# mathwrx/Decouple-and-Couple_Learning_in_Multi-Modal_Brain_Tumor_Segmentation

Hardware: AMD Instinct MI355X
Metric: training volumes/sec (4x128^3) (higher is better)
Workload: dtype bf16x3 forward (split-bf16 MFMA operands hi.hi+hi.lo+lo.hi: logits within 1e-3 of the fp32 reference) / bf16 data-gradient / bf16 weight-gradient MFMA operands; f32 accumulate, f32 storage, f32 master weights

## Files before the change

### decouple-and-couple_learning_in_multi-modal_brain_tumor_segmentation_amd/csrc/conv_args.h

```cpp
#pragma once
#include "common.h"

typedef __bf16 bf16x8 __attribute__((ext_vector_type(8)));
typedef unsigned u32x4 __attribute__((ext_vector_type(4)));

struct ConvArgsB {
  ConvGeom g;
  const float* x; const uint4* wpk; const float* bias; float* y;
  const float* in_scale; const float* in_shift; float in_slope;
  const float* residual; int r_ldc; const float* out_scale; double* stats;
  unsigned long long unused_[2];
  const float* nb_x; int nb_ldc; const float* nb_scale; const float* nb_shift; float nb_slope;
  int groups, x_goff, y_goff;
  const uint4* wpk_g[3]; const float* bias_g[3];
  const uint4* x16; const uint4* zero16;
  unsigned short* y16;
};

typedef __bf16 bf16x2_t __attribute__((ext_vector_type(2)));
typedef float f32x2_t __attribute__((ext_vector_type(2)));
__device__ __forceinline__ unsigned pack_bf16(float a, float b) {
  const f32x2_t f = {a, b};
  return __builtin_bit_cast(unsigned, __builtin_convertvector(f, bf16x2_t));
}
__device__ __forceinline__ float bf16_round(float a) { return (float)(__bf16)a; }
__device__ __forceinline__ void split_bf16(float a, float b, unsigned& hi, unsigned& lo) {
  hi = pack_bf16(a, b);
  const float ha = __builtin_bit_cast(float, hi << 16), hb = __builtin_bit_cast(float, hi & 0xffff0000u);
  lo = pack_bf16(a - ha, b - hb);
}
__device__ __forceinline__ float act01(float v, float slope) { return fmaxf(v, v * slope); }


static inline int cfg_extent(int op, int Di, int Hi, int Wi, int Do, int Ho, int Wo, int cd[3]) {
  cd[0] = Do; cd[1] = Ho; cd[2] = Wo;
  if (op == CWF_CONVT2) { cd[0] = Di; cd[1] = Hi; cd[2] = Wi; return 8; }
  if (op == CWF_CONV3_S2_DGRAD) { cd[0] = (Do + 1) / 2; cd[1] = (Ho + 1) / 2; cd[2] = (Wo + 1) / 2; return 8; }
  return 1;
}

int cwf_try_conv_ws(int op, int x3, ConvArgsB& a, hipStream_t st, int* rc);
int cwf_ws_takes_x3();
int cwf_try_conv_wsp(int op, int x3, int cfg_mt, int cfg_wm, ConvArgsB& a, hipStream_t st, int* rc);

int conv_fp32_launch(const cwf_conv_args& d, hipStream_t st);
int conv_stem_launch(const cwf_conv_args& d, hipStream_t st);
int conv_s2c16_launch(const cwf_conv_args& d, hipStream_t st);
int wgrad_fp32_launch(const cwf_wgrad_args& d, int* nsplit_used, hipStream_t st);
```

### decouple-and-couple_learning_in_multi-modal_brain_tumor_segmentation_amd/csrc/conv_ws.hip

```cpp
#include "conv_args.h"
#include <cstdlib>
#include <type_traits>

#define WS_ID 6
#define WS_IH 6
#define WS_IW 18
#define WS_NVOX (WS_ID * WS_IH * WS_IW)
#define WS_SLOTS 11
#define WS_NT 2

struct WsWork { int ngroups, slots, tiles, xcd_perm; };

__host__ __device__ constexpr int ws_tap_bytes(int t) { return (((t / 9) * WS_IH + (t / 3) % 3) * WS_IW + t % 3) * 32; }

template <bool X3>
__global__ __launch_bounds__(512) void convws_kernel(const ConvArgsB a, const WsWork wk) {
  constexpr int NT = WS_NT;
  constexpr int T = 1;
  extern __shared__ float4 lds4[];
  const ConvGeom& g = a.g;
  const int nch = g.nchunks;
  char* lds = reinterpret_cast<char*>(lds4);
  constexpr int B_IMG = 14 * NT * 1024;
  constexpr int B_ALL = B_IMG * (X3 ? 2 : 1);
  constexpr int A_IMG = WS_NVOX * 32;
  constexpr int A_GRP = A_IMG * (X3 ? 2 : 1);
  constexpr int NB = (B_ALL + 4095) / 4096;
  char* Bh = lds;
  char* Bl = lds + B_IMG;
  const int tid = threadIdx.x, lane = tid & 63;
  const int wave = __builtin_amdgcn_readfirstlane(tid >> 6);
  const int grp = wave >> 2, wl = wave & 3, tg = tid & 255;
  char* Ah = lds + B_ALL + grp * A_GRP;
  char* Al = Ah + A_IMG;
  float* red = reinterpret_cast<float*>(lds + B_ALL + 2 * A_GRP);
  const int r = lane & 15, kq = lane >> 4;
  const bool second = (kq >> 1) != 0;

  int cgrp, slot;
  {
    const int b = blockIdx.x;
    if (wk.xcd_perm) {
      const int per = gridDim.x >> 3, j = b >> 3;
      cgrp = j % wk.ngroups;
      slot = (b & 7) * (per / wk.ngroups) + j / wk.ngroups;
    } else {
      cgrp = b % wk.ngroups;
      slot = b / wk.ngroups;
    }
  }
  const int t_begin = (int)(((int64_t)slot * wk.tiles) / wk.slots), t_end = (int)(((int64_t)(slot + 1) * wk.tiles) / wk.slots);
  const int nt0 = cgrp * NT;
  const int n_rounds = (t_end - t_begin + 2 * T - 1) / (2 * T);
  const int n_blocks = n_rounds * nch;
  const int tiles_per_n = g.tiles_d * g.tiles_h * g.tiles_w;
  auto item_tile = [&](int round, int k) { const int t = t_begin + round * 2 * T + 2 * k + grp; return t < t_end ? t : -1; };

  u32x4 bpf[NB];
  const uint4* wsrc = a.wpk + (int64_t)g.cls_wbase16[0] * 128;
  auto b_issue = [&](int chunk) {
    int tgo = tg;
    asm volatile("" : "+v"(tgo));
#pragma unroll
    for (int i = 0; i < NB; ++i) {
      int e = tgo + 256 * i;
      if (e >= B_ALL / 16) e = 0;
      const int img = e / (14 * NT * 64), e2 = e % (14 * NT * 64);
      const int ln = e2 & 63, blk = e2 >> 6;
      const int j = blk % NT, s = blk / NT;
      const uint4* p = wsrc + ((int64_t)(chunk * 14 + s) * g.ntiles + nt0 + j) * 128 + ln * 2 + img;
      bpf[i] = *reinterpret_cast<const u32x4*>(p);
    }
  };
  auto b_write = [&]() {
    int wb = tg * 16;
    asm volatile("" : "+v"(wb));
#pragma unroll
    for (int i = 0; i < NB; ++i)
      if (256 * (i + 1) <= B_ALL / 16 || tg + 256 * i < B_ALL / 16) *reinterpret_cast<u32x4*>(Bh + wb + i * 4096) = bpf[i];
  };

  const int q = tg & 3;
  const int vox0 = tg >> 2;
  const int iw_0 = vox0 % WS_IW, row_0 = vox0 / WS_IW;
  const bool plain = a.in_scale == nullptr && a.in_slope == 1.f;

  f32x4 pf[WS_SLOTS];
  f32x4 pf_sc, pf_sh;
  unsigned pf_inb = 0u;
  auto issue_loads = [&](int tile, int chunk) {
    const int n = tile / tiles_per_n;
    int bx = tile - n * tiles_per_n;
    const int tw = bx % g.tiles_w; bx /= g.tiles_w;
    const int th = bx % g.tiles_h, td = bx / g.tiles_h;
    const int id0 = td * 4 - 1, ih0 = th * 4 - 1, iw0 = tw * 16 - 1;
    const float* xb = a.x + (int64_t)n * g.Di * g.Hi * g.Wi * g.x_ldc + chunk * 16;
    const unsigned ldc4 = (unsigned)g.x_ldc * 4u;
    pf_inb = 0u;
    int iw = iw_0, row = row_0;
    asm volatile("" : "+v"(iw), "+v"(row));
#pragma unroll
    for (int i = 0; i < WS_SLOTS; ++i) {
      const int idd = (row * 43) >> 8, ih = row - idd * WS_IH;
      const int gd = id0 + idd, gh = ih0 + ih, gw = iw0 + iw;
      const bool ok = (row < WS_ID * WS_IH) & ((unsigned)gd < (unsigned)g.Di) & ((unsigned)gh < (unsigned)g.Hi) & ((unsigned)gw < (unsigned)g.Wi);
      iw += 10; row += 3;
      if (iw >= WS_IW) { iw -= WS_IW; ++row; }
      const unsigned lin = (unsigned)((gd * g.Hi + gh) * g.Wi + gw) * ldc4 + (unsigned)q * 16u;
      const unsigned boff = ok ? lin : (unsigned)q * 16u;
      pf[i] = *reinterpret_cast<const f32x4*>(reinterpret_cast<const char*>(xb) + boff);
      pf_inb |= ok ? (1u << i) : 0u;
    }
    const float* scp = a.in_scale ? a.in_scale + (int64_t)n * g.Cin + chunk * 16 : a.x;
    const float* shp = a.in_scale ? a.in_shift + (int64_t)n * g.Cin + chunk * 16 : a.x;
    const unsigned qo = (unsigned)q * 16u;
    pf_sc = *reinterpret_cast<const f32x4*>(reinterpret_cast<const char*>(scp) + qo);
    pf_sh = *reinterpret_cast<const f32x4*>(reinterpret_cast<const char*>(shp) + qo);
  };
  auto convert_write = [&](int tile, int chunk, const f32x4& sc, const f32x4& sh) {
    const float slope = a.in_slope;
    int vbase = (tg >> 2) * 32 + q * 8;
    asm volatile("" : "+v"(vbase));
#pragma unroll
    for (int i = 0; i < WS_SLOTS; ++i) {
      if (i == WS_SLOTS - 1 && vox0 + 64 * i >= WS_NVOX) continue;
      float v0 = pf[i][0], v1 = pf[i][1], v2 = pf[i][2], v3 = pf[i][3];
      if (!plain) {
        v0 = act01(fmaf(v0, sc[0], sh[0]), slope); v1 = act01(fmaf(v1, sc[1], sh[1]), slope);
        v2 = act01(fmaf(v2, sc[2], sh[2]), slope); v3 = act01(fmaf(v3, sc[3], sh[3]), slope);
      }
      uint2 h, l;
      if (X3) { split_bf16(v0, v1, h.x, l.x); split_bf16(v2, v3, h.y, l.y); }
      else { h.x = pack_bf16(v0, v1); h.y = pack_bf16(v2, v3); l = make_uint2(0u, 0u); }
      const bool was = (pf_inb >> i) & 1u;
      h.x = was ? h.x : 0u; h.y = was ? h.y : 0u; l.x = was ? l.x : 0u; l.y = was ? l.y : 0u;
      *reinterpret_cast<uint2*>(Ah + vbase + i * (64 * 32)) = h;
      if (X3) *reinterpret_cast<uint2*>(Al + vbase + i * (64 * 32)) = l;
    }
  };

  const int a_lane = ((wl * WS_IH) * WS_IW + r) * 32 + (kq & 1) * 16;
  const int b_lane = lane * 16;

  f32x4 acc[T][4][NT];
#pragma unroll
  for (int k = 0; k < T; ++k)
#pragma unroll
    for (int m = 0; m < 4; ++m)
#pragma unroll
      for (int j = 0; j < NT; ++j) acc[k][m][j] = (f32x4){0.f, 0.f, 0.f, 0.f};
  float s1[NT], s2[NT];
#pragma unroll
  for (int j = 0; j < NT; ++j) { s1[j] = 0.f; s2[j] = 0.f; }
  int stats_n = -1;

  auto flush_stats_wave = [&]() {
#pragma unroll
    for (int j = 0; j < NT; ++j) {
      float u1 = s1[j], u2 = s2[j];
      u1 += __shfl_xor(u1, 16, 64); u1 += __shfl_xor(u1, 32, 64);
      u2 += __shfl_xor(u2, 16, 64); u2 += __shfl_xor(u2, 32, 64);
      if (kq == 0) {
        const int co = (nt0 + j) * 16 + r;
        atomic_add_f64(a.stats + ((int64_t)stats_n * g.Cout + co) * 2 + 0, (double)u1);
        atomic_add_f64(a.stats + ((int64_t)stats_n * g.Cout + co) * 2 + 1, (double)u2);
      }
      s1[j] = 0.f; s2[j] = 0.f;
    }
  };

  auto epilogue = [&](int tile, auto KK) {
    constexpr int k = decltype(KK)::value;
    const int n = tile / tiles_per_n;
    int bx = tile - n * tiles_per_n;
    const int tw = bx % g.tiles_w; bx /= g.tiles_w;
    const int th = bx % g.tiles_h, td = bx / g.tiles_h;
    if (a.stats && n != stats_n) {
      if (stats_n >= 0) flush_stats_wave();
      stats_n = n;
    }
    float bvj[NT];
#pragma unroll
    for (int j = 0; j < NT; ++j) bvj[j] = a.bias ? a.bias[(nt0 + j) * 16 + r] : 0.f;
    auto epi = [&](auto HR, auto HT, auto HN) {
      constexpr bool HAS_RES = decltype(HR)::value, HAS_STATS = decltype(HT)::value, HAS_NB = decltype(HN)::value;
      unsigned yo[4], ro[4], xo[4];
      float nsc[NT], nsh[NT];
#pragma unroll
      for (int i = 0; i < 4; ++i) {
        yo[i] = (unsigned)((kq * 4 + i) * g.y_ldc + nt0 * 16 + r) * 4u; asm volatile("" : "+v"(yo[i]));
        if (HAS_RES) { ro[i] = (unsigned)((kq * 4 + i) * a.r_ldc + nt0 * 16 + r) * 4u; asm volatile("" : "+v"(ro[i])); }
        if (HAS_NB) { xo[i] = (unsigned)((kq * 4 + i) * a.nb_ldc + nt0 * 16 + r) * 4u; asm volatile("" : "+v"(xo[i])); }
      }
      if (HAS_NB) {
#pragma unroll
        for (int j = 0; j < NT; ++j) {
          nsc[j] = a.nb_scale[(int64_t)n * g.Cout + (nt0 + j) * 16 + r];
          nsh[j] = a.nb_shift[(int64_t)n * g.Cout + (nt0 + j) * 16 + r];
        }
      }
#pragma unroll
      for (int m = 0; m < 4; ++m) {
        const int od = td * 4 + wl, oh = th * 4 + m;
        const int64_t vox0 = (((int64_t)n * g.Do + od) * g.Ho + oh) * g.Wo + tw * 16;
        char* yb = reinterpret_cast<char*>(a.y + vox0 * g.y_ldc);
        const char* rb = HAS_RES ? reinterpret_cast<const char*>(a.residual + vox0 * a.r_ldc) : nullptr;
        const char* xb = HAS_NB ? reinterpret_cast<const char*>(a.nb_x + vox0 * a.nb_ldc) : nullptr;
        float rv[NT][4], xv[NT][4];
        if (HAS_RES) {
#pragma unroll
          for (int j = 0; j < NT; ++j)
#pragma unroll
            for (int i = 0; i < 4; ++i) rv[j][i] = *reinterpret_cast<const float*>(rb + ro[i] + j * 64);
        }
        if (HAS_NB) {
#pragma unroll
          for (int j = 0; j < NT; ++j)
#pragma unroll
            for (int i = 0; i < 4; ++i) xv[j][i] = *reinterpret_cast<const float*>(xb + xo[i] + j * 64);
        }
#pragma unroll
        for (int j = 0; j < NT; ++j)
#pragma unroll
          for (int i = 0; i < 4; ++i) {
            float v = acc[k][m][j][i] + bvj[j];
            if (HAS_RES) v += rv[j][i];
            *reinterpret_cast<float*>(yb + yo[i] + j * 64) = v;
            if (HAS_NB) {
              const float h = fmaf(xv[j][i], nsc[j], nsh[j]);
              const float gn = v * (h > 0.f ? 1.f : a.nb_slope);
              s1[j] += gn; s2[j] = fmaf(gn, h, s2[j]);
            } else if (HAS_STATS) { s1[j] += v; s2[j] = fmaf(v, v, s2[j]); }
            acc[k][m][j][i] = 0.f;
          }
      }
    };
    using T_ = std::true_type; using F_ = std::false_type;
    if (a.nb_x) { if (a.residual) epi(T_{}, T_{}, T_{}); else epi(F_{}, T_{}, T_{}); }
    else if (a.residual) { if (a.stats) epi(T_{}, T_{}, F_{}); else epi(T_{}, F_{}, F_{}); }
    else            { if (a.stats) epi(F_{}, T_{}, F_{}); else epi(F_{}, F_{}, F_{}); }
  };

  auto mfma_item = [&](int block, auto KK) -> bool {
    constexpr int k = decltype(KK)::value;
    const int round = block / nch, chunk = block - round * nch;
    const int tile = item_tile(round, k);
    if (tile < 0) return false;
    const char* bh = Bh + b_lane;
    const char* bl = Bl + b_lane;
    const char* ah0 = Ah + a_lane;
    const char* al0 = Al + a_lane;
    uint4 fa[2][4], fb[2][NT], fl[4], fbl[NT];
    auto rd_hi = [&](auto S, auto P) {
      constexpr int s = decltype(S)::value, p = decltype(P)::value;
      constexpr int c0 = ws_tap_bytes(2 * s), c1 = ws_tap_bytes(2 * s + 1 < 27 ? 2 * s + 1 : 2 * s);
      const int to = second ? c1 : c0;
#pragma unroll
      for (int m = 0; m < 4; ++m) fa[p][m] = *reinterpret_cast<const uint4*>(ah0 + to + m * (WS_IW * 32));
#pragma unroll
      for (int j = 0; j < NT; ++j) fb[p][j] = *reinterpret_cast<const uint4*>(bh + (s * NT + j) * 1024);
    };
    auto rd_lo = [&](auto S) {
      constexpr int s = decltype(S)::value;
      constexpr int c0 = ws_tap_bytes(2 * s), c1 = ws_tap_bytes(2 * s + 1 < 27 ? 2 * s + 1 : 2 * s);
      const int to = second ? c1 : c0;
#pragma unroll
      for (int m = 0; m < 4; ++m) fl[m] = *reinterpret_cast<const uint4*>(al0 + to + m * (WS_IW * 32));
#pragma unroll
      for (int j = 0; j < NT; ++j) fbl[j] = *reinterpret_cast<const uint4*>(bl + (s * NT + j) * 1024);
    };
    auto mm = [&](auto P) {
      constexpr int p = decltype(P)::value;
#pragma unroll
      for (int m = 0; m < 4; ++m)
#pragma unroll
        for (int j = 0; j < NT; ++j)
          acc[k][m][j] = __builtin_amdgcn_mfma_f32_16x16x32_bf16(__builtin_bit_cast(bf16x8, fa[p][m]), __builtin_bit_cast(bf16x8, fb[p][j]), acc[k][m][j], 0, 0, 0);
      if (X3) {
#pragma unroll
        for (int m = 0; m < 4; ++m)
#pragma unroll
          for (int j = 0; j < NT; ++j)
            acc[k][m][j] = __builtin_amdgcn_mfma_f32_16x16x32_bf16(__builtin_bit_cast(bf16x8, fa[p][m]), __builtin_bit_cast(bf16x8, fbl[j]), acc[k][m][j], 0, 0, 0);
#pragma unroll
        for (int m = 0; m < 4; ++m)
#pragma unroll
          for (int j = 0; j < NT; ++j)
            acc[k][m][j] = __builtin_amdgcn_mfma_f32_16x16x32_bf16(__builtin_bit_cast(bf16x8, fl[m]), __builtin_bit_cast(bf16x8, fb[p][j]), acc[k][m][j], 0, 0, 0);
      }
    };
    using I0 = std::integral_constant<int, 0>; using I1 = std::integral_constant<int, 1>;
#define WS_IC(v) std::integral_constant<int, (v)>{}
#define WS_STEP2(S0)                                                                                           \
    if (X3) rd_lo(WS_IC(S0)); rd_hi(WS_IC((S0) + 1), I1{}); mm(I0{}); __builtin_amdgcn_sched_barrier(0);       \
    if (X3) rd_lo(WS_IC((S0) + 1)); if ((S0) + 2 < 14) rd_hi(WS_IC((S0) + 2 < 14 ? (S0) + 2 : 13), I0{});      \
    mm(I1{}); __builtin_amdgcn_sched_barrier(0);
    rd_hi(I0{}, I0{});
    WS_STEP2(0) WS_STEP2(2) WS_STEP2(4) WS_STEP2(6) WS_STEP2(8) WS_STEP2(10) WS_STEP2(12)
#undef WS_STEP2
#undef WS_IC
    if (chunk == nch - 1) { epilogue(tile, KK); return true; }
    return false;
  };
  using K0 = std::integral_constant<int, 0>;
  auto do_issue = [&](int blk) {
    const int round = blk / nch, tile = item_tile(round, 0);
    if (tile >= 0) issue_loads(tile, blk - round * nch);
  };
  auto do_convert = [&](int blk, int younger) {
    const int round = blk / nch, tile = item_tile(round, 0);
    if (tile < 0) return;
    (void)younger;
    asm volatile("" : "+v"(pf_sc), "+v"(pf_sh));
    convert_write(tile, blk - round * nch, pf_sc, pf_sh);
  };
  if (n_blocks > 0) {
    do_issue(0);
    if (grp == 0) {
      b_issue(0);
      do_convert(0, -1);
      __syncthreads();
      b_write();
      __syncthreads();
      for (int blk = 0; blk < n_blocks; ++blk) {
        const bool more = blk + 1 < n_blocks;
        if (more) do_issue(blk + 1);
        const bool epi = mfma_item(blk, K0{});
        __syncthreads();
        if (more) {
          b_issue((blk + 1) % nch);
          do_convert(blk + 1, NB + (epi ? 32 : 0));
        }
        __syncthreads();
        if (more) {
          b_write();
          __syncthreads();
        }
      }
    } else {
      __syncthreads();
      __syncthreads();
      do_convert(0, -1);
      for (int blk = 0; blk < n_blocks; ++blk) {
        const bool more = blk + 1 < n_blocks;
        __syncthreads();
        if (more) do_issue(blk + 1);
        const bool epi = mfma_item(blk, K0{});
        __syncthreads();
        if (more) {
          __syncthreads();
          do_convert(blk + 1, epi ? 32 : 0);
        }
      }
    }
  }

  if (a.stats) {
#pragma unroll
    for (int j = 0; j < NT; ++j) {
      float u1 = s1[j], u2 = s2[j];
      u1 += __shfl_xor(u1, 16, 64); u1 += __shfl_xor(u1, 32, 64);
      u2 += __shfl_xor(u2, 16, 64); u2 += __shfl_xor(u2, 32, 64);
      if (kq == 0) {
        red[((wave * NT + j) * 16 + r) * 2 + 0] = u1;
        red[((wave * NT + j) * 16 + r) * 2 + 1] = u2;
      }
    }
    int* red_n = reinterpret_cast<int*>(red + 8 * NT * 16 * 2);
    if (lane == 0) red_n[wave] = stats_n;
    __syncthreads();
    if (tid < 2 * NT * 16 * 2) {
      const int gsel = tid / (NT * 16 * 2), t2 = tid % (NT * 16 * 2);
      const int which = t2 & 1, rr = (t2 >> 1) & 15, jj = t2 >> 5;
      const int sn = red_n[gsel * 4];
      if (sn >= 0) {
        double s = 0.0;
#pragma unroll
        for (int w = 0; w < 4; ++w) s += (double)red[(((gsel * 4 + w) * NT + jj) * 16 + rr) * 2 + which];
        const int co = (nt0 + jj) * 16 + rr;
        atomic_add_f64(a.stats + ((int64_t)sn * g.Cout + co) * 2 + which, s);
      }
    }
  }
}

namespace {
template <bool X3>
int launch_ws(const ConvArgsB& a, const WsWork& wk, int grid, hipStream_t st) {
  const size_t lds = (size_t)14 * WS_NT * 1024 * (X3 ? 2 : 1) + (size_t)2 * WS_NVOX * 32 * (X3 ? 2 : 1) + 8 * WS_NT * 16 * 2 * sizeof(float) + 64;
  if (lds > 160 * 1024) return CWF_E_TOOLARGE;
  CWF_MAX_LDS_ONCE((&convws_kernel<X3>));
  hipLaunchKernelGGL((convws_kernel<X3>), dim3(grid), dim3(512), lds, st, a, wk);
  CWF_LAUNCH_CHECK();
  return 0;
}
}

static int g_ws_min_units = 256;
extern "C" int cwf_debug_ws_min_units(int v) { const int old = g_ws_min_units; g_ws_min_units = v; return old; }
static int g_ws_x3 = 0;
extern "C" int cwf_debug_ws_x3(int v) { const int old = g_ws_x3; g_ws_x3 = v; return old; }
int cwf_ws_takes_x3() { return g_ws_x3; }

int cwf_try_conv_ws(int op, int x3, ConvArgsB& a, hipStream_t st, int* rc) {
  const ConvGeom& g = a.g;
  if (op != CWF_CONV3_S1 || a.groups || a.out_scale || (x3 && !g_ws_x3)) return 0;
  if (g.Cin < 32 || (g.Cin & 15) || (g.Cout & 31)) return 0;
  if ((g.Do & 3) || (g.Ho & 3) || (g.Wo & 15)) return 0;
  if (g.x_ldc < g.Cin || (g.x_ldc & 3)) return 0;
  WsWork wk;
  wk.ngroups = g.Cout / 32;
  if (wk.ngroups > 32) return 0;
  const int64_t tiles = (int64_t)g.N * (g.Do / 4) * (g.Ho / 4) * (g.Wo / 16);
  if (tiles * wk.ngroups < g_ws_min_units) return 0;
  int e = cwf_build_geom(a.g, op, g.N, g.Di, g.Hi, g.Wi, g.Cin, g.x_ldc, g.Do, g.Ho, g.Wo, g.Cout, g.y_ldc, 16);
  if (e) { *rc = e; return 1; }
  wk.tiles = (int)tiles;
  int per = (32 / wk.ngroups) * wk.ngroups;
  wk.slots = 8 * (per / wk.ngroups);
  wk.xcd_perm = 1;
  if (wk.slots * 2 > wk.tiles) { wk.slots = (wk.tiles + 1) / 2; wk.xcd_perm = 0; }
  const int grid = wk.slots * wk.ngroups;
  *rc = x3 ? launch_ws<true>(a, wk, grid, st) : launch_ws<false>(a, wk, grid, st);
  return 1;
}
```

### decouple-and-couple_learning_in_multi-modal_brain_tumor_segmentation_amd/csrc/conv_wsp.hip

```cpp
#include "conv_args.h"
#include <cstdlib>
#include <type_traits>

#define WSP_ID 6
#define WSP_IH 6
#define WSP_IW 18
#define WSP_NVOX (WSP_ID * WSP_IH * WSP_IW)
#define WSP_SLOTS 11
#define WSP_NT 2
#define WSP_NBW 14

struct WspWork { int ngroups, slots, tiles, xcd_perm, stat_rows; };

__host__ __device__ constexpr int wsp_tap_bytes(int t) { return (((t / 9) * WSP_IH + (t / 3) % 3) * WSP_IW + t % 3) * 32; }

template <int T>
__global__ __launch_bounds__(512) void convwsp_kernel(const ConvArgsB a, const WspWork wk) {
  constexpr int NT = WSP_NT;
  constexpr int B_IMG = 14 * NT * 1024;
  constexpr int A_IMG = WSP_NVOX * 32;
  constexpr int A_BUF = 2 * A_IMG;
  extern __shared__ float4 lds4[];
  char* lds = reinterpret_cast<char*>(lds4);
  char* const Bh = lds;
  char* const Bl = lds + B_IMG;
  char* const A0 = lds + 2 * B_IMG;
  const ConvGeom& g = a.g;
  const int nch = g.nchunks;
  const int tid = threadIdx.x, lane = tid & 63;
  const int wave = __builtin_amdgcn_readfirstlane(tid >> 6);

  int cgrp, slot;
  {
    const int b = blockIdx.x;
    if (wk.xcd_perm) {
      const int per = gridDim.x >> 3, j = b >> 3;
      cgrp = j % wk.ngroups;
      slot = (b & 7) * (per / wk.ngroups) + j / wk.ngroups;
    } else {
      cgrp = b % wk.ngroups;
      slot = b / wk.ngroups;
    }
  }
  const int t_begin = (int)(((int64_t)slot * wk.tiles) / wk.slots), t_end = (int)(((int64_t)(slot + 1) * wk.tiles) / wk.slots);
  const int ntw = t_end - t_begin;
  const int nt0 = cgrp * NT;
  const int tiles_per_n = g.tiles_d * g.tiles_h * g.tiles_w;

  if (wave < 4) {
    const int wl = wave;
    const int r = lane & 15, kq = lane >> 4;
    const bool second = (kq >> 1) != 0;
    const int a_lane = ((wl * WSP_IH) * WSP_IW + r) * 32 + (kq & 1) * 16;
    const int b_lane = lane * 16;

    f32x4 acc[T][4][NT];
#pragma unroll
    for (int k = 0; k < T; ++k)
#pragma unroll
      for (int m = 0; m < 4; ++m)
#pragma unroll
        for (int j = 0; j < NT; ++j) acc[k][m][j] = (f32x4){0.f, 0.f, 0.f, 0.f};
    float s1[NT], s2[NT];
    double d1[NT], d2[NT];
#pragma unroll
    for (int j = 0; j < NT; ++j) { s1[j] = 0.f; s2[j] = 0.f; d1[j] = 0.0; d2[j] = 0.0; }
    int stats_n = -1;
    auto fold_stats = [&]() {
#pragma unroll
      for (int j = 0; j < NT; ++j) {
        float u1 = s1[j], u2 = s2[j];
        u1 += __shfl_xor(u1, 16, 64); u1 += __shfl_xor(u1, 32, 64);
        u2 += __shfl_xor(u2, 16, 64); u2 += __shfl_xor(u2, 32, 64);
        d1[j] += (double)u1; d2[j] += (double)u2;
        s1[j] = 0.f; s2[j] = 0.f;
      }
    };
    auto flush_stats = [&]() {
#pragma unroll
      for (int j = 0; j < NT; ++j) {
        if (kq == 0) {
          const int co = (nt0 + j) * 16 + r;
          atomic_add_f64(a.stats + ((int64_t)stats_n * g.Cout + co) * 2 + 0, d1[j]);
          atomic_add_f64(a.stats + ((int64_t)stats_n * g.Cout + co) * 2 + 1, d2[j]);
        }
        d1[j] = 0.0; d2[j] = 0.0;
      }
    };

    auto epilogue = [&](int tile, auto KK) {
      constexpr int k = decltype(KK)::value;
      const int n = tile / tiles_per_n;
      int bx = tile - n * tiles_per_n;
      const int tw = bx % g.tiles_w; bx /= g.tiles_w;
      const int th = bx % g.tiles_h, td = bx / g.tiles_h;
      if (a.stats && n != stats_n) {
        if (stats_n >= 0) flush_stats();
        stats_n = n;
      }
      float bvj[NT];
#pragma unroll
      for (int j = 0; j < NT; ++j) bvj[j] = a.bias ? a.bias[(nt0 + j) * 16 + r] : 0.f;
      auto epi = [&](auto HR, auto HT) {
        constexpr bool HAS_RES = decltype(HR)::value, HAS_STATS = decltype(HT)::value;
        unsigned yo[4], ro[4];
#pragma unroll
        for (int i = 0; i < 4; ++i) {
          yo[i] = (unsigned)((kq * 4 + i) * g.y_ldc + nt0 * 16 + r) * 4u; asm volatile("" : "+v"(yo[i]));
          if (HAS_RES) { ro[i] = (unsigned)((kq * 4 + i) * a.r_ldc + nt0 * 16 + r) * 4u; asm volatile("" : "+v"(ro[i])); }
        }
        const int od = td * 4 + wl;
        float rv[4][NT][4];
        if (HAS_RES) {
#pragma unroll
          for (int m = 0; m < 4; ++m) {
            const int64_t vox0 = (((int64_t)n * g.Do + od) * g.Ho + th * 4 + m) * g.Wo + tw * 16;
            const char* rb = reinterpret_cast<const char*>(a.residual + vox0 * a.r_ldc);
#pragma unroll
            for (int j = 0; j < NT; ++j)
#pragma unroll
              for (int i = 0; i < 4; ++i) rv[m][j][i] = *reinterpret_cast<const float*>(rb + ro[i] + j * 64);
          }
        }
#pragma unroll
        for (int m = 0; m < 4; ++m) {
          const int64_t vox0 = (((int64_t)n * g.Do + od) * g.Ho + th * 4 + m) * g.Wo + tw * 16;
          char* yb = reinterpret_cast<char*>(a.y + vox0 * g.y_ldc);
#pragma unroll
          for (int j = 0; j < NT; ++j)
#pragma unroll
            for (int i = 0; i < 4; ++i) {
              float v = acc[k][m][j][i] + bvj[j];
              if (HAS_RES) v += rv[m][j][i];
              *reinterpret_cast<float*>(yb + yo[i] + j * 64) = v;
              if (HAS_STATS) { s1[j] += v; s2[j] = fmaf(v, v, s2[j]); }
              acc[k][m][j][i] = 0.f;
            }
          if (HAS_STATS && (wk.stat_rows == 1 || m == 3)) fold_stats();
        }
      };
      using T_ = std::true_type; using F_ = std::false_type;
      if (a.residual) { if (a.stats) epi(T_{}, T_{}); else epi(T_{}, F_{}); }
      else            { if (a.stats) epi(F_{}, T_{}); else epi(F_{}, F_{}); }
    };

    auto mfma_item = [&](int buf, auto KK) {
      constexpr int k = decltype(KK)::value;
      const char* bh = Bh + b_lane;
      const char* bl = Bl + b_lane;
      const char* ah0 = A0 + buf * A_BUF + a_lane;
      const char* al0 = ah0 + A_IMG;
      uint4 fa[2][4], fb[2][NT], fl[4], fbl[NT];
      auto rd_hi = [&](auto S, auto P) {
        constexpr int s = decltype(S)::value, p = decltype(P)::value;
        constexpr int c0 = wsp_tap_bytes(2 * s), c1 = wsp_tap_bytes(2 * s + 1 < 27 ? 2 * s + 1 : 2 * s);
        const int to = second ? c1 : c0;
#pragma unroll
        for (int m = 0; m < 4; ++m) fa[p][m] = *reinterpret_cast<const uint4*>(ah0 + to + m * (WSP_IW * 32));
#pragma unroll
        for (int j = 0; j < NT; ++j) fb[p][j] = *reinterpret_cast<const uint4*>(bh + (s * NT + j) * 1024);
      };
      auto rd_lo = [&](auto S) {
        constexpr int s = decltype(S)::value;
        constexpr int c0 = wsp_tap_bytes(2 * s), c1 = wsp_tap_bytes(2 * s + 1 < 27 ? 2 * s + 1 : 2 * s);
        const int to = second ? c1 : c0;
#pragma unroll
        for (int m = 0; m < 4; ++m) fl[m] = *reinterpret_cast<const uint4*>(al0 + to + m * (WSP_IW * 32));
#pragma unroll
        for (int j = 0; j < NT; ++j) fbl[j] = *reinterpret_cast<const uint4*>(bl + (s * NT + j) * 1024);
      };
      auto mm = [&](auto P) {
        constexpr int p = decltype(P)::value;
#pragma unroll
        for (int m = 0; m < 4; ++m)
#pragma unroll
          for (int j = 0; j < NT; ++j)
            acc[k][m][j] = __builtin_amdgcn_mfma_f32_16x16x32_bf16(__builtin_bit_cast(bf16x8, fa[p][m]), __builtin_bit_cast(bf16x8, fb[p][j]), acc[k][m][j], 0, 0, 0);
#pragma unroll
        for (int m = 0; m < 4; ++m)
#pragma unroll
          for (int j = 0; j < NT; ++j)
            acc[k][m][j] = __builtin_amdgcn_mfma_f32_16x16x32_bf16(__builtin_bit_cast(bf16x8, fa[p][m]), __builtin_bit_cast(bf16x8, fbl[j]), acc[k][m][j], 0, 0, 0);
#pragma unroll
        for (int m = 0; m < 4; ++m)
#pragma unroll
          for (int j = 0; j < NT; ++j)
            acc[k][m][j] = __builtin_amdgcn_mfma_f32_16x16x32_bf16(__builtin_bit_cast(bf16x8, fl[m]), __builtin_bit_cast(bf16x8, fb[p][j]), acc[k][m][j], 0, 0, 0);
      };
      using I0 = std::integral_constant<int, 0>; using I1 = std::integral_constant<int, 1>;
#define WSP_IC(v) std::integral_constant<int, (v)>{}
#define WSP_STEP2(S0)                                                                                          \
      rd_lo(WSP_IC(S0)); rd_hi(WSP_IC((S0) + 1), I1{}); mm(I0{}); __builtin_amdgcn_sched_barrier(0);            \
      rd_lo(WSP_IC((S0) + 1)); if ((S0) + 2 < 14) rd_hi(WSP_IC((S0) + 2 < 14 ? (S0) + 2 : 13), I0{});           \
      mm(I1{}); __builtin_amdgcn_sched_barrier(0);
      rd_hi(I0{}, I0{});
      WSP_STEP2(0) WSP_STEP2(2) WSP_STEP2(4) WSP_STEP2(6) WSP_STEP2(8) WSP_STEP2(10) WSP_STEP2(12)
#undef WSP_STEP2
#undef WSP_IC
    };

    int i = 0;
    for (int t0 = 0; t0 < ntw; t0 += T) {
      const int nk = min(T, ntw - t0);
      for (int c = 0; c < nch; ++c) {
        auto item = [&](auto KK) {
          constexpr int k = decltype(KK)::value;
          if (k == 0 && i > 0) asm volatile("s_barrier" ::: "memory");
          asm volatile("s_barrier" ::: "memory");
          mfma_item(i & 1, KK);
          if (c == nch - 1) epilogue(t_begin + t0 + k, KK);
          ++i;
        };
        item(std::integral_constant<int, 0>{});
        if (T > 1 && nk > 1) item(std::integral_constant<int, (T > 1 ? 1 : 0)>{});
        if (T > 2 && nk > 2) item(std::integral_constant<int, (T > 2 ? 2 : 0)>{});
        if (T > 3 && nk > 3) item(std::integral_constant<int, (T > 3 ? 3 : 0)>{});
      }
    }
    if (a.stats && stats_n >= 0) flush_stats();
  } else {
    const int tg = tid - 256;
    const int ni = ntw * nch;
    struct Item { int tile, chunk; bool first; };
    auto item_of = [&](int it) {
      const int per_round = T * nch;
      const int rd = it / per_round, w = it - rd * per_round;
      const int nk = min(T, ntw - rd * T);
      const int c = w / nk, k = w - c * nk;
      Item o; o.tile = t_begin + rd * T + k; o.chunk = c; o.first = k == 0;
      return o;
    };

    u32x4 wpf[WSP_NBW];
    const uint4* wsrc = a.wpk + (int64_t)g.cls_wbase16[0] * 128;
    auto w_issue = [&](int chunk) {
      int tgo = tg;
      asm volatile("" : "+v"(tgo));
#pragma unroll
      for (int i = 0; i < WSP_NBW; ++i) {
        const int e = tgo + 256 * i;
        const int img = e / (14 * NT * 64), e2 = e - img * (14 * NT * 64);
        const int ln = e2 & 63, blk = e2 >> 6;
        const int j = blk % NT, s = blk / NT;
        const uint4* p = wsrc + ((int64_t)(chunk * 14 + s) * g.ntiles + nt0 + j) * 128 + ln * 2 + img;
        wpf[i] = *reinterpret_cast<const u32x4*>(p);
      }
    };
    auto w_write = [&]() {
      int wb = tg * 16;
      asm volatile("" : "+v"(wb));
#pragma unroll
      for (int i = 0; i < WSP_NBW; ++i) *reinterpret_cast<u32x4*>(Bh + wb + i * 4096) = wpf[i];
    };

    const int q = tg & 3;
    const int vox0 = tg >> 2;
    const int iw_0 = vox0 % WSP_IW, row_0 = vox0 / WSP_IW;
    const bool plain = a.in_scale == nullptr && a.in_slope == 1.f;
    f32x4 pf[WSP_SLOTS];
    f32x4 pf_sc, pf_sh;
    unsigned pf_inb = 0u;
    auto issue = [&](int it) {
      const Item itm = item_of(it);
      const int tile = itm.tile, chunk = itm.chunk;
      const int n = tile / tiles_per_n;
      int bx = tile - n * tiles_per_n;
      const int tw = bx % g.tiles_w; bx /= g.tiles_w;
      const int th = bx % g.tiles_h, td = bx / g.tiles_h;
      const int id0 = td * 4 - 1, ih0 = th * 4 - 1, iw0 = tw * 16 - 1;
      const char* xb = reinterpret_cast<const char*>(a.x + (int64_t)n * g.Di * g.Hi * g.Wi * g.x_ldc + chunk * 16);
      const unsigned ldc4 = (unsigned)g.x_ldc * 4u;
      unsigned inb = 0u;
      int iw = iw_0, row = row_0;
      asm volatile("" : "+v"(iw), "+v"(row));
#pragma unroll
      for (int i = 0; i < WSP_SLOTS; ++i) {
        const int idd = (row * 43) >> 8, ih = row - idd * WSP_IH;
        const int gd = id0 + idd, gh = ih0 + ih, gw = iw0 + iw;
        const bool ok = (row < WSP_ID * WSP_IH) & ((unsigned)gd < (unsigned)g.Di) & ((unsigned)gh < (unsigned)g.Hi) & ((unsigned)gw < (unsigned)g.Wi);
        iw += 10; row += 3;
        if (iw >= WSP_IW) { iw -= WSP_IW; ++row; }
        const unsigned lin = (unsigned)((gd * g.Hi + gh) * g.Wi + gw) * ldc4 + (unsigned)q * 16u;
        const unsigned boff = ok ? lin : (unsigned)q * 16u;
        pf[i] = *reinterpret_cast<const f32x4*>(xb + boff);
        inb |= ok ? (1u << i) : 0u;
      }
      pf_inb = inb;
      const float* scp = a.in_scale ? a.in_scale + (int64_t)n * g.Cin + chunk * 16 : a.x;
      const float* shp = a.in_scale ? a.in_shift + (int64_t)n * g.Cin + chunk * 16 : a.x;
      pf_sc = *reinterpret_cast<const f32x4*>(reinterpret_cast<const char*>(scp) + q * 16);
      pf_sh = *reinterpret_cast<const f32x4*>(reinterpret_cast<const char*>(shp) + q * 16);
    };
    auto convert = [&](int buf) {
      const float slope = a.in_slope;
      const bool has_norm = a.in_scale != nullptr;
      const f32x4 sc = has_norm ? pf_sc : (f32x4){1.f, 1.f, 1.f, 1.f}, sh = has_norm ? pf_sh : (f32x4){0.f, 0.f, 0.f, 0.f};
      const unsigned inb = pf_inb;
      int vbase = (tg >> 2) * 32 + q * 8;
      asm volatile("" : "+v"(vbase));
      char* ah = A0 + buf * A_BUF + vbase;
#pragma unroll
      for (int i = 0; i < WSP_SLOTS; ++i) {
        if (i == WSP_SLOTS - 1 && vox0 + 64 * i >= WSP_NVOX) continue;
        float v0 = pf[i][0], v1 = pf[i][1], v2 = pf[i][2], v3 = pf[i][3];
        if (!plain) {
          v0 = act01(fmaf(v0, sc[0], sh[0]), slope); v1 = act01(fmaf(v1, sc[1], sh[1]), slope);
          v2 = act01(fmaf(v2, sc[2], sh[2]), slope); v3 = act01(fmaf(v3, sc[3], sh[3]), slope);
        }
        uint2 h, l;
        split_bf16(v0, v1, h.x, l.x); split_bf16(v2, v3, h.y, l.y);
        const bool was = (inb >> i) & 1u;
        h.x = was ? h.x : 0u; h.y = was ? h.y : 0u; l.x = was ? l.x : 0u; l.y = was ? l.y : 0u;
        *reinterpret_cast<uint2*>(ah + i * (64 * 32)) = h;
        *reinterpret_cast<uint2*>(ah + A_IMG + i * (64 * 32)) = l;
      }
    };

    __builtin_amdgcn_s_setprio(1);
    if (ni > 0) {
      issue(0);
      w_issue(0);
      convert(0);
      w_write();
      if (ni > 1) issue(1);
    }
    for (int it = 0; it < ni; ++it) {
      if (it > 0 && item_of(it).first) {
        asm volatile("s_barrier" ::: "memory");
        w_write();
      }
      asm volatile("s_waitcnt lgkmcnt(0)\n\ts_barrier" ::: "memory");
      if (it + 1 < ni) {
        convert((it + 1) & 1);
        const Item nx = item_of(it + 1);
        if (nx.first) w_issue(nx.chunk);
        if (it + 2 < ni) issue(it + 2);
      }
    }
  }
}

namespace {
template <int T>
int launch_wsp(const ConvArgsB& a, const WspWork& wk, int grid, hipStream_t st) {
  const size_t lds = (size_t)2 * 14 * WSP_NT * 1024 + (size_t)2 * 2 * WSP_NVOX * 32;
  CWF_MAX_LDS_ONCE((&convwsp_kernel<T>));
  hipLaunchKernelGGL((convwsp_kernel<T>), dim3(grid), dim3(512), lds, st, a, wk);
  CWF_LAUNCH_CHECK();
  return 0;
}
}

static int g_wsp = 1;
extern "C" int cwf_debug_wsp(int v) { const int old = g_wsp; g_wsp = v; return old; }
static long long g_wsp_launches = 0;
extern "C" long long cwf_debug_wsp_launches() { return g_wsp_launches; }
static const int g_wsp_min_cin = 128, g_wsp_min_units = 128;

int cwf_try_conv_wsp(int op, int x3, int cfg_mt, int cfg_wm, ConvArgsB& a, hipStream_t st, int* rc) {
  const ConvGeom& g = a.g;
  if (!g_wsp || !x3 || cwf_ws_takes_x3()) return 0;
  if (op != CWF_CONV3_S1 || a.groups || a.out_scale || a.nb_x) return 0;
  if (g.Cin < 32 || (g.Cin & 15) || (g.Cout & 31)) return 0;
  if ((g.Do & 3) || (g.Ho & 3) || (g.Wo & 15)) return 0;
  if (g.x_ldc < g.Cin || (g.x_ldc & 3)) return 0;
  if ((int64_t)g.Di * g.Hi * g.Wi * g.x_ldc * 4 >= (1ll << 31)) return 0;
  if (a.stats && !(cfg_mt == 1 || (cfg_mt == 4 && cfg_wm == 4))) return 0;
  WspWork wk;
  wk.stat_rows = cfg_mt;
  wk.ngroups = g.Cout / 32;
  if (wk.ngroups > 32) return 0;
  const int64_t tiles = (int64_t)g.N * (g.Do / 4) * (g.Ho / 4) * (g.Wo / 16);
  if (g_wsp == 1 && (g.Cin < g_wsp_min_cin || tiles * wk.ngroups < g_wsp_min_units)) return 0;
  int e = cwf_build_geom(a.g, op, g.N, g.Di, g.Hi, g.Wi, g.Cin, g.x_ldc, g.Do, g.Ho, g.Wo, g.Cout, g.y_ldc, 16);
  if (e) { *rc = e; return 1; }
  wk.tiles = (int)tiles;
  const int per = (32 / wk.ngroups) * wk.ngroups;
  wk.slots = 8 * (per / wk.ngroups);
  wk.xcd_perm = 1;
  if (wk.slots > wk.tiles) { wk.slots = wk.tiles; wk.xcd_perm = 0; }
  const int grid = wk.slots * wk.ngroups;
  const int per_wg = (wk.tiles + wk.slots - 1) / wk.slots;
  *rc = per_wg > 2 ? launch_wsp<4>(a, wk, grid, st) : launch_wsp<2>(a, wk, grid, st);
  if (*rc == 0) ++g_wsp_launches;
  return 1;
}
```

Measured before the change: 115.3.

## Extend warp-specialized conv to single-bf16 path with LDS-resident weights and fused stats

```diff
diff --git a/decouple-and-couple_learning_in_multi-modal_brain_tumor_segmentation_amd/csrc/conv_args.h b/decouple-and-couple_learning_in_multi-modal_brain_tumor_segmentation_amd/csrc/conv_args.h
--- a/decouple-and-couple_learning_in_multi-modal_brain_tumor_segmentation_amd/csrc/conv_args.h
+++ b/decouple-and-couple_learning_in_multi-modal_brain_tumor_segmentation_amd/csrc/conv_args.h
@@ -41,6 +41,7 @@
 
 int cwf_try_conv_ws(int op, int x3, ConvArgsB& a, hipStream_t st, int* rc);
 int cwf_ws_takes_x3();
+int cwf_ws_min_units();
 int cwf_try_conv_wsp(int op, int x3, int cfg_mt, int cfg_wm, ConvArgsB& a, hipStream_t st, int* rc);
 
 int conv_fp32_launch(const cwf_conv_args& d, hipStream_t st);
diff --git a/decouple-and-couple_learning_in_multi-modal_brain_tumor_segmentation_amd/csrc/conv_ws.hip b/decouple-and-couple_learning_in_multi-modal_brain_tumor_segmentation_amd/csrc/conv_ws.hip
--- a/decouple-and-couple_learning_in_multi-modal_brain_tumor_segmentation_amd/csrc/conv_ws.hip
+++ b/decouple-and-couple_learning_in_multi-modal_brain_tumor_segmentation_amd/csrc/conv_ws.hip
@@ -401,6 +401,7 @@
 static int g_ws_x3 = 0;
 extern "C" int cwf_debug_ws_x3(int v) { const int old = g_ws_x3; g_ws_x3 = v; return old; }
 int cwf_ws_takes_x3() { return g_ws_x3; }
+int cwf_ws_min_units() { return g_ws_min_units; }
 
 int cwf_try_conv_ws(int op, int x3, ConvArgsB& a, hipStream_t st, int* rc) {
   const ConvGeom& g = a.g;
diff --git a/decouple-and-couple_learning_in_multi-modal_brain_tumor_segmentation_amd/csrc/conv_wsp.hip b/decouple-and-couple_learning_in_multi-modal_brain_tumor_segmentation_amd/csrc/conv_wsp.hip
--- a/decouple-and-couple_learning_in_multi-modal_brain_tumor_segmentation_amd/csrc/conv_wsp.hip
+++ b/decouple-and-couple_learning_in_multi-modal_brain_tumor_segmentation_amd/csrc/conv_wsp.hip
@@ -14,19 +14,24 @@
 
 __host__ __device__ constexpr int wsp_tap_bytes(int t) { return (((t / 9) * WSP_IH + (t / 3) % 3) * WSP_IW + t % 3) * 32; }
 
-template <int T>
+template <int T, bool X3, bool RES>
 __global__ __launch_bounds__(512) void convwsp_kernel(const ConvArgsB a, const WspWork wk) {
+  static_assert(!(X3 && RES), "resident weights: single bf16 only");
   constexpr int NT = WSP_NT;
+  constexpr int NIMG = X3 ? 2 : 1;
   constexpr int B_IMG = 14 * NT * 1024;
   constexpr int A_IMG = WSP_NVOX * 32;
-  constexpr int A_BUF = 2 * A_IMG;
+  constexpr int A_BUF = NIMG * A_IMG;
+  constexpr int NBW = WSP_NBW / (X3 ? 1 : 2);
+  constexpr bool PRE = !X3 && (RES || T <= 2);
   extern __shared__ float4 lds4[];
   char* lds = reinterpret_cast<char*>(lds4);
+  const ConvGeom& g = a.g;
+  const int nch = g.nchunks;
   char* const Bh = lds;
   char* const Bl = lds + B_IMG;
-  char* const A0 = lds + 2 * B_IMG;
-  const ConvGeom& g = a.g;
-  const int nch = g.nchunks;
+  char* const A0 = lds + (RES ? nch : NIMG) * B_IMG;
+  double* const red = reinterpret_cast<double*>(A0 + 2 * A_BUF);
   const int tid = threadIdx.x, lane = tid & 63;
   const int wave = __builtin_amdgcn_readfirstlane(tid >> 6);
 
@@ -66,6 +71,10 @@
 #pragma unroll
     for (int j = 0; j < NT; ++j) { s1[j] = 0.f; s2[j] = 0.f; d1[j] = 0.0; d2[j] = 0.0; }
     int stats_n = -1;
+    float o1[NT], o2[NT];
+#pragma unroll
+    for (int j = 0; j < NT; ++j) { o1[j] = 0.f; o2[j] = 0.f; }
+    int ostats_n = -1;
     auto fold_stats = [&]() {
 #pragma unroll
       for (int j = 0; j < NT; ++j) {
@@ -85,6 +94,40 @@
           atomic_add_f64(a.stats + ((int64_t)stats_n * g.Cout + co) * 2 + 1, d2[j]);
         }
         d1[j] = 0.0; d2[j] = 0.0;
+      }
+    };
+
+    struct EpiOps { float rv[4][NT][4], xv[4][NT][4]; };
+    EpiOps pre;
+    auto load_epi = [&](EpiOps& eo, int tile, bool has_res, bool has_nb) {
+      const int n = tile / tiles_per_n;
+      int bx = tile - n * tiles_per_n;
+      const int tw = bx % g.tiles_w; bx /= g.tiles_w;
+      const int th = bx % g.tiles_h, td = bx / g.tiles_h;
+      const int od = td * 4 + wl;
+      unsigned ro[4], xo[4];
+#pragma unroll
+      for (int i = 0; i < 4; ++i) {
+        ro[i] = (unsigned)((kq * 4 + i) * a.r_ldc + nt0 * 16 + r) * 4u; asm volatile("" : "+v"(ro[i]));
+        xo[i] = (unsigned)((kq * 4 + i) * a.nb_ldc + nt0 * 16 + r) * 4u; asm volatile("" : "+v"(xo[i]));
+      }
+#pragma unroll
+      for (int m = 0; m < 4; ++m) {
+        const int64_t vox0 = (((int64_t)n * g.Do + od) * g.Ho + th * 4 + m) * g.Wo + tw * 16;
+        if (has_res) {
+          const char* rb = reinterpret_cast<const char*>(a.residual + vox0 * a.r_ldc);
+#pragma unroll
+          for (int j = 0; j < NT; ++j)
+#pragma unroll
+            for (int i = 0; i < 4; ++i) eo.rv[m][j][i] = *reinterpret_cast<const float*>(rb + ro[i] + j * 64);
+        }
+        if (has_nb) {
+          const char* xb = reinterpret_cast<const char*>(a.nb_x + vox0 * a.nb_ldc);
+#pragma unroll
+          for (int j = 0; j < NT; ++j)
+#pragma unroll
+            for (int i = 0; i < 4; ++i) eo.xv[m][j][i] = *reinterpret_cast<const float*>(xb + xo[i] + j * 64);
+        }
       }
     };
 
@@ -95,33 +138,31 @@
       const int tw = bx % g.tiles_w; bx /= g.tiles_w;
       const int th = bx % g.tiles_h, td = bx / g.tiles_h;
       if (a.stats && n != stats_n) {
-        if (stats_n >= 0) flush_stats();
+        if (stats_n >= 0) { if (wk.stat_rows == 0) fold_stats(); flush_stats(); }
         stats_n = n;
       }
       float bvj[NT];
 #pragma unroll
       for (int j = 0; j < NT; ++j) bvj[j] = a.bias ? a.bias[(nt0 + j) * 16 + r] : 0.f;
-      auto epi = [&](auto HR, auto HT) {
-        constexpr bool HAS_RES = decltype(HR)::value, HAS_STATS = decltype(HT)::value;
-        unsigned yo[4], ro[4];
+      auto epi = [&](auto HR, auto HT, auto HN) {
+        constexpr bool HAS_RES = decltype(HR)::value, HAS_STATS = decltype(HT)::value, HAS_NB = decltype(HN)::value;
+        unsigned yo[4];
+        float nsc[NT], nsh[NT];
 #pragma unroll
         for (int i = 0; i < 4; ++i) {
           yo[i] = (unsigned)((kq * 4 + i) * g.y_ldc + nt0 * 16 + r) * 4u; asm volatile("" : "+v"(yo[i]));
-          if (HAS_RES) { ro[i] = (unsigned)((kq * 4 + i) * a.r_ldc + nt0 * 16 + r) * 4u; asm volatile("" : "+v"(ro[i])); }
+        }
+        if (HAS_NB) {
+#pragma unroll
+          for (int j = 0; j < NT; ++j) {
+            nsc[j] = a.nb_scale[(int64_t)n * g.Cout + (nt0 + j) * 16 + r];
+            nsh[j] = a.nb_shift[(int64_t)n * g.Cout + (nt0 + j) * 16 + r];
+          }
         }
         const int od = td * 4 + wl;
-        float rv[4][NT][4];
-        if (HAS_RES) {
-#pragma unroll
-          for (int m = 0; m < 4; ++m) {
-            const int64_t vox0 = (((int64_t)n * g.Do + od) * g.Ho + th * 4 + m) * g.Wo + tw * 16;
-            const char* rb = reinterpret_cast<const char*>(a.residual + vox0 * a.r_ldc);
-#pragma unroll
-            for (int j = 0; j < NT; ++j)
-#pragma unroll
-              for (int i = 0; i < 4; ++i) rv[m][j][i] = *reinterpret_cast<const float*>(rb + ro[i] + j * 64);
-          }
-        }
+        EpiOps loc;
+        if (!PRE) load_epi(loc, tile, HAS_RES, HAS_NB);
+        const EpiOps& eo = PRE ? pre : loc;
 #pragma unroll
         for (int m = 0; m < 4; ++m) {
           const int64_t vox0 = (((int64_t)n * g.Do + od) * g.Ho + th * 4 + m) * g.Wo + tw * 16;
@@ -131,22 +172,35 @@
 #pragma unroll
             for (int i = 0; i < 4; ++i) {
               float v = acc[k][m][j][i] + bvj[j];
-              if (HAS_RES) v += rv[m][j][i];
+              if (HAS_RES) v += eo.rv[m][j][i];
               *reinterpret_cast<float*>(yb + yo[i] + j * 64) = v;
-              if (HAS_STATS) { s1[j] += v; s2[j] = fmaf(v, v, s2[j]); }
+              if (HAS_NB) {
+                const float h = fmaf(eo.xv[m][j][i], nsc[j], nsh[j]);
+                const float gn = v * (h > 0.f ? 1.f : a.nb_slope);
+                s1[j] += gn; s2[j] = fmaf(gn, h, s2[j]);
+              } else if (HAS_STATS) { s1[j] += v; s2[j] = fmaf(v, v, s2[j]); }
               acc[k][m][j][i] = 0.f;
             }
-          if (HAS_STATS && (wk.stat_rows == 1 || m == 3)) fold_stats();
+          if (HAS_STATS && wk.stat_rows != 0 && (wk.stat_rows == 1 || m == 3)) fold_stats();
         }
       };
       using T_ = std::true_type; using F_ = std::false_type;
-      if (a.residual) { if (a.stats) epi(T_{}, T_{}); else epi(T_{}, F_{}); }
-      else            { if (a.stats) epi(F_{}, T_{}); else epi(F_{}, F_{}); }
-    };
-
-    auto mfma_item = [&](int buf, auto KK) {
+      if (!X3 && a.nb_x) { if (a.residual) epi(T_{}, T_{}, T_{}); else epi(F_{}, T_{}, T_{}); }
+      else if (a.residual) { if (a.stats) epi(T_{}, T_{}, F_{}); else epi(T_{}, F_{}, F_{}); }
+      else            { if (a.stats) epi(F_{}, T_{}, F_{}); else epi(F_{}, F_{}, F_{}); }
+      if (a.stats && wk.stat_rows == 0) {
+#pragma unroll
+        for (int j = 0; j < NT; ++j) {
+          const float t1 = s1[j], t2 = s2[j];
+          s1[j] = o1[j]; s2[j] = o2[j]; o1[j] = t1; o2[j] = t2;
+        }
+        const int tn = stats_n; stats_n = ostats_n; ostats_n = tn;
+      }
+    };
+
+    auto mfma_item = [&](int buf, auto KK, int wchunk) {
       constexpr int k = decltype(KK)::value;
-      const char* bh = Bh + b_lane;
+      const char* bh = Bh + b_lane + (RES ? wchunk * B_IMG : 0);
       const char* bl = Bl + b_lane;
       const char* ah0 = A0 + buf * A_BUF + a_lane;
       const char* al0 = ah0 + A_IMG;
@@ -176,22 +230,24 @@
 #pragma unroll
           for (int j = 0; j < NT; ++j)
             acc[k][m][j] = __builtin_amdgcn_mfma_f32_16x16x32_bf16(__builtin_bit_cast(bf16x8, fa[p][m]), __builtin_bit_cast(bf16x8, fb[p][j]), acc[k][m][j], 0, 0, 0);
-#pragma unroll
-        for (int m = 0; m < 4; ++m)
-#pragma unroll
-          for (int j = 0; j < NT; ++j)
-            acc[k][m][j] = __builtin_amdgcn_mfma_f32_16x16x32_bf16(__builtin_bit_cast(bf16x8, fa[p][m]), __builtin_bit_cast(bf16x8, fbl[j]), acc[k][m][j], 0, 0, 0);
-#pragma unroll
-        for (int m = 0; m < 4; ++m)
-#pragma unroll
-          for (int j = 0; j < NT; ++j)
-            acc[k][m][j] = __builtin_amdgcn_mfma_f32_16x16x32_bf16(__builtin_bit_cast(bf16x8, fl[m]), __builtin_bit_cast(bf16x8, fb[p][j]), acc[k][m][j], 0, 0, 0);
+        if constexpr (X3) {
+#pragma unroll
+          for (int m = 0; m < 4; ++m)
+#pragma unroll
+            for (int j = 0; j < NT; ++j)
+              acc[k][m][j] = __builtin_amdgcn_mfma_f32_16x16x32_bf16(__builtin_bit_cast(bf16x8, fa[p][m]), __builtin_bit_cast(bf16x8, fbl[j]), acc[k][m][j], 0, 0, 0);
+#pragma unroll
+          for (int m = 0; m < 4; ++m)
+#pragma unroll
+            for (int j = 0; j < NT; ++j)
+              acc[k][m][j] = __builtin_amdgcn_mfma_f32_16x16x32_bf16(__builtin_bit_cast(bf16x8, fl[m]), __builtin_bit_cast(bf16x8, fb[p][j]), acc[k][m][j], 0, 0, 0);
+        }
       };
       using I0 = std::integral_constant<int, 0>; using I1 = std::integral_constant<int, 1>;
 #define WSP_IC(v) std::integral_constant<int, (v)>{}
 #define WSP_STEP2(S0)                                                                                          \
-      rd_lo(WSP_IC(S0)); rd_hi(WSP_IC((S0) + 1), I1{}); mm(I0{}); __builtin_amdgcn_sched_barrier(0);            \
-      rd_lo(WSP_IC((S0) + 1)); if ((S0) + 2 < 14) rd_hi(WSP_IC((S0) + 2 < 14 ? (S0) + 2 : 13), I0{});           \
+      if constexpr (X3) rd_lo(WSP_IC(S0)); rd_hi(WSP_IC((S0) + 1), I1{}); mm(I0{}); __builtin_amdgcn_sched_barrier(0); \
+      if constexpr (X3) rd_lo(WSP_IC((S0) + 1)); if ((S0) + 2 < 14) rd_hi(WSP_IC((S0) + 2 < 14 ? (S0) + 2 : 13), I0{});           \
       mm(I1{}); __builtin_amdgcn_sched_barrier(0);
       rd_hi(I0{}, I0{});
       WSP_STEP2(0) WSP_STEP2(2) WSP_STEP2(4) WSP_STEP2(6) WSP_STEP2(8) WSP_STEP2(10) WSP_STEP2(12)
@@ -200,6 +256,17 @@
     };
 
     int i = 0;
+    if constexpr (RES) {
+      using K0 = std::integral_constant<int, 0>;
+      for (int t = 0; t < ntw; ++t)
+        for (int c = 0; c < nch; ++c) {
+          asm volatile("s_barrier" ::: "memory");
+          if (c == 0) load_epi(pre, t_begin + t, a.residual != nullptr, a.nb_x != nullptr);
+          mfma_item(i & 1, K0{}, c);
+          if (c == nch - 1) epilogue(t_begin + t, K0{});
+          ++i;
+        }
+    } else {
     for (int t0 = 0; t0 < ntw; t0 += T) {
       const int nk = min(T, ntw - t0);
       for (int c = 0; c < nch; ++c) {
@@ -207,7 +274,8 @@
           constexpr int k = decltype(KK)::value;
           if (k == 0 && i > 0) asm volatile("s_barrier" ::: "memory");
           asm volatile("s_barrier" ::: "memory");
-          mfma_item(i & 1, KK);
+          if (PRE && c == nch - 1) load_epi(pre, t_begin + t0 + k, a.residual != nullptr, a.nb_x != nullptr);
+          mfma_item(i & 1, KK, 0);
           if (c == nch - 1) epilogue(t_begin + t0 + k, KK);
           ++i;
         };
@@ -217,12 +285,43 @@
         if (T > 3 && nk > 3) item(std::integral_constant<int, (T > 3 ? 3 : 0)>{});
       }
     }
-    if (a.stats && stats_n >= 0) flush_stats();
+    }
+    if (a.stats) {
+      if (wk.stat_rows == 0) {
+        if (stats_n >= 0) fold_stats();
+        const int cur_n = stats_n;
+        if (ostats_n >= 0 && cur_n >= 0 && ostats_n != cur_n) flush_stats();
+#pragma unroll
+        for (int j = 0; j < NT; ++j) { s1[j] = o1[j]; s2[j] = o2[j]; }
+        stats_n = ostats_n >= 0 ? ostats_n : cur_n;
+        if (ostats_n >= 0) fold_stats();
+      }
+      if (kq == 0) {
+#pragma unroll
+        for (int j = 0; j < NT; ++j) {
+          red[((wl * NT + j) * 16 + r) * 2 + 0] = d1[j];
+          red[((wl * NT + j) * 16 + r) * 2 + 1] = d2[j];
+        }
+      }
+      asm volatile("s_waitcnt lgkmcnt(0)\n\ts_barrier" ::: "memory");
+      if (wl == 0 && stats_n >= 0) {
+        const int which = lane & 1, rr = (lane >> 1) & 15, jj = lane >> 5;
+        double sum = 0.0;
+#pragma unroll
+        for (int w = 0; w < 4; ++w) sum += red[((w * NT + jj) * 16 + rr) * 2 + which];
+        atomic_add_f64(a.stats + ((int64_t)stats_n * g.Cout + (nt0 + jj) * 16 + rr) * 2 + which, sum);
+      }
+    }
   } else {
     const int tg = tid - 256;
     const int ni = ntw * nch;
     struct Item { int tile, chunk; bool first; };
     auto item_of = [&](int it) {
+      if constexpr (RES) {
+        const int t = it / nch;
+        Item o; o.tile = t_begin + t; o.chunk = it - t * nch; o.first = false;
+        return o;
+      }
       const int per_round = T * nch;
       const int rd = it / per_round, w = it - rd * per_round;
       const int nk = min(T, ntw - rd * T);
@@ -231,13 +330,13 @@
       return o;
     };
 
-    u32x4 wpf[WSP_NBW];
+    u32x4 wpf[NBW];
     const uint4* wsrc = a.wpk + (int64_t)g.cls_wbase16[0] * 128;
     auto w_issue = [&](int chunk) {
       int tgo = tg;
       asm volatile("" : "+v"(tgo));
 #pragma unroll
-      for (int i = 0; i < WSP_NBW; ++i) {
+      for (int i = 0; i < NBW; ++i) {
         const int e = tgo + 256 * i;
         const int img = e / (14 * NT * 64), e2 = e - img * (14 * NT * 64);
         const int ln = e2 & 63, blk = e2 >> 6;
@@ -246,11 +345,11 @@
         wpf[i] = *reinterpret_cast<const u32x4*>(p);
       }
     };
-    auto w_write = [&]() {
-      int wb = tg * 16;
+    auto w_write = [&](int slot = 0) {
+      int wb = tg * 16 + slot * B_IMG;
       asm volatile("" : "+v"(wb));
 #pragma unroll
-      for (int i = 0; i < WSP_NBW; ++i) *reinterpret_cast<u32x4*>(Bh + wb + i * 4096) = wpf[i];
+      for (int i = 0; i < NBW; ++i) *reinterpret_cast<u32x4*>(Bh + wb + i * 4096) = wpf[i];
     };
 
     const int q = tg & 3;
@@ -308,11 +407,12 @@
           v2 = act01(fmaf(v2, sc[2], sh[2]), slope); v3 = act01(fmaf(v3, sc[3], sh[3]), slope);
         }
         uint2 h, l;
-        split_bf16(v0, v1, h.x, l.x); split_bf16(v2, v3, h.y, l.y);
+        if constexpr (X3) { split_bf16(v0, v1, h.x, l.x); split_bf16(v2, v3, h.y, l.y); }
+        else { h.x = pack_bf16(v0, v1); h.y = pack_bf16(v2, v3); l = make_uint2(0u, 0u); }
         const bool was = (inb >> i) & 1u;
         h.x = was ? h.x : 0u; h.y = was ? h.y : 0u; l.x = was ? l.x : 0u; l.y = was ? l.y : 0u;
         *reinterpret_cast<uint2*>(ah + i * (64 * 32)) = h;
-        *reinterpret_cast<uint2*>(ah + A_IMG + i * (64 * 32)) = l;
+        if constexpr (X3) *reinterpret_cast<uint2*>(ah + A_IMG + i * (64 * 32)) = l;
       }
     };
 
@@ -322,6 +422,8 @@
       w_issue(0);
       convert(0);
       w_write();
+      if constexpr (RES)
+        for (int c = 1; c < nch; ++c) { w_issue(c); w_write(c); }
       if (ni > 1) issue(1);
     }
     for (int it = 0; it < ni; ++it) {
@@ -337,15 +439,18 @@
         if (it + 2 < ni) issue(it + 2);
       }
     }
+    if (a.stats) asm volatile("s_barrier" ::: "memory");
   }
 }
 
 namespace {
-template <int T>
+template <int T, bool X3, bool RES>
 int launch_wsp(const ConvArgsB& a, const WspWork& wk, int grid, hipStream_t st) {
-  const size_t lds = (size_t)2 * 14 * WSP_NT * 1024 + (size_t)2 * 2 * WSP_NVOX * 32;
-  CWF_MAX_LDS_ONCE((&convwsp_kernel<T>));
-  hipLaunchKernelGGL((convwsp_kernel<T>), dim3(grid), dim3(512), lds, st, a, wk);
+  const size_t lds = (size_t)(RES ? a.g.nchunks : (X3 ? 2 : 1)) * 14 * WSP_NT * 1024 + (size_t)2 * (X3 ? 2 : 1) * WSP_NVOX * 32 +
+                     4 * WSP_NT * 16 * 2 * sizeof(double);
+  if (lds > 160 * 1024) return CWF_E_TOOLARGE;
+  CWF_MAX_LDS_ONCE((&convwsp_kernel<T, X3, RES>));
+  hipLaunchKernelGGL((convwsp_kernel<T, X3, RES>), dim3(grid), dim3(512), lds, st, a, wk);
   CWF_LAUNCH_CHECK();
   return 0;
 }
@@ -356,32 +461,44 @@
 static long long g_wsp_launches = 0;
 extern "C" long long cwf_debug_wsp_launches() { return g_wsp_launches; }
 static const int g_wsp_min_cin = 128, g_wsp_min_units = 128;
+static const int g_wsp1_res_min_units = 256, g_wsp1_max_cin = 256;
 
 int cwf_try_conv_wsp(int op, int x3, int cfg_mt, int cfg_wm, ConvArgsB& a, hipStream_t st, int* rc) {
   const ConvGeom& g = a.g;
-  if (!g_wsp || !x3 || cwf_ws_takes_x3()) return 0;
-  if (op != CWF_CONV3_S1 || a.groups || a.out_scale || a.nb_x) return 0;
+  if (!g_wsp || (x3 && cwf_ws_takes_x3())) return 0;
+  if (op != CWF_CONV3_S1 || a.groups || a.out_scale || (x3 && a.nb_x)) return 0;
   if (g.Cin < 32 || (g.Cin & 15) || (g.Cout & 31)) return 0;
   if ((g.Do & 3) || (g.Ho & 3) || (g.Wo & 15)) return 0;
   if (g.x_ldc < g.Cin || (g.x_ldc & 3)) return 0;
   if ((int64_t)g.Di * g.Hi * g.Wi * g.x_ldc * 4 >= (1ll << 31)) return 0;
-  if (a.stats && !(cfg_mt == 1 || (cfg_mt == 4 && cfg_wm == 4))) return 0;
   WspWork wk;
-  wk.stat_rows = cfg_mt;
   wk.ngroups = g.Cout / 32;
   if (wk.ngroups > 32) return 0;
   const int64_t tiles = (int64_t)g.N * (g.Do / 4) * (g.Ho / 4) * (g.Wo / 16);
-  if (g_wsp == 1 && (g.Cin < g_wsp_min_cin || tiles * wk.ngroups < g_wsp_min_units)) return 0;
+  const bool from_ws = !x3 && tiles * wk.ngroups >= cwf_ws_min_units();
+  if (!from_ws && a.stats && !(cfg_mt == 1 || (cfg_mt == 4 && cfg_wm == 4))) return 0;
+  wk.stat_rows = from_ws ? 0 : cfg_mt;
+  const int nch = g.Cin / 16;
+  const bool res = !x3 && (size_t)nch * 14 * WSP_NT * 1024 + (size_t)2 * WSP_NVOX * 32 + 2048 <= 160 * 1024;
+  if (g_wsp == 1) {
+    if (x3 && (g.Cin < g_wsp_min_cin || tiles * wk.ngroups < g_wsp_min_units)) return 0;
+    if (!x3 && !(res ? tiles * wk.ngroups >= g_wsp1_res_min_units
+                     : g.Cin >= g_wsp_min_cin && g.Cin <= g_wsp1_max_cin && tiles * wk.ngroups >= g_wsp_min_units)) return 0;
+  }
   int e = cwf_build_geom(a.g, op, g.N, g.Di, g.Hi, g.Wi, g.Cin, g.x_ldc, g.Do, g.Ho, g.Wo, g.Cout, g.y_ldc, 16);
   if (e) { *rc = e; return 1; }
   wk.tiles = (int)tiles;
   const int per = (32 / wk.ngroups) * wk.ngroups;
   wk.slots = 8 * (per / wk.ngroups);
   wk.xcd_perm = 1;
-  if (wk.slots > wk.tiles) { wk.slots = wk.tiles; wk.xcd_perm = 0; }
+  if (from_ws) {
+    if (wk.slots * 2 > wk.tiles) { wk.slots = (wk.tiles + 1) / 2; wk.xcd_perm = 0; }
+  } else if (wk.slots > wk.tiles) { wk.slots = wk.tiles; wk.xcd_perm = 0; }
   const int grid = wk.slots * wk.ngroups;
   const int per_wg = (wk.tiles + wk.slots - 1) / wk.slots;
-  *rc = per_wg > 2 ? launch_wsp<4>(a, wk, grid, st) : launch_wsp<2>(a, wk, grid, st);
+  if (x3) *rc = per_wg > 2 ? launch_wsp<4, true, false>(a, wk, grid, st) : launch_wsp<2, true, false>(a, wk, grid, st);
+  else if (res) *rc = launch_wsp<1, false, true>(a, wk, grid, st);
+  else *rc = launch_wsp<2, false, false>(a, wk, grid, st);
   if (*rc == 0) ++g_wsp_launches;
   return 1;
 }
```

Result: faster. 116.8 (median of 6 runs) (+1.3%).
